# LiWentomng/BoxInstSeg

Measured on AMD Instinct MI355X. Metric: pairwise+projection loss fwd+bwd images/sec @2x800x1024x32inst, higher is better.
Workload: dtype f32; 1 GPU; BoxInst R-50 FPN loss path, 2x800x1024 synthetic batch, 32 instances, 1xMI355X per rank (BASELINE configs[1]); instances=32, launch=eager, input_sets=8, parallelism=replicas x1 (no exchange step inside the path)

## Files before the change

### boxinstseg_amd/csrc/fused_eval.hip

```cpp
#include "loss_common.hpp"
#include "dynamic_head_device.hpp"
#include <algorithm>
#include <atomic>
#include <cstdlib>
#include <cstring>
#include <cmath>
#include <ctime>

namespace bxi {

constexpr int kWaves = 4;
constexpr int kSRows = 8;
constexpr int kSBlk = kWaves * kSRows;
constexpr int kChunkC = 256;
constexpr int kMaxDilFused = 4;
#ifndef BXI_SPIN_LIMIT
#define BXI_SPIN_LIMIT 4000000
#endif
constexpr int kSpinLimit = BXI_SPIN_LIMIT;
constexpr unsigned kFlagSingle = BXI_EVAL_SINGLE_LAUNCH, kFlagTwo = BXI_EVAL_TWO_LAUNCHES, kFlagRows8 = BXI_EVAL_TILE_ROWS_8, kFlagRows4 = BXI_EVAL_TILE_ROWS_4,
                   kFlagShared = BXI_EVAL_SHARED_DEVICE, kFlagTargetsReady = BXI_EVAL_TARGETS_READY, kFlagGiveUp = BXI_EVAL_WAITS_GIVE_UP;
constexpr int kBoxCap = 1024;
constexpr int kBoxSplit = 8;
constexpr int kNtStreamFromMB = 20;
constexpr int kLongFrom = 96;
constexpr unsigned int kMaxTag = 0x0fffffffu;
constexpr int kAcc2Split = 8, kAcc2Stride = 16;
constexpr int kAcc1Words = 64;
constexpr int kMaxInst = 65536;
constexpr int kOneOcc = 4;
constexpr int kLongOcc = 3;
constexpr int kPrepOcc = 5;
#ifdef BXI_WAITLOG
static __device__ unsigned int g_waitlog[16];
#define BXI_WL(site, spins) do { if ((spins) > 1000 && (threadIdx.x & 63) == 0) atomicMax(&g_waitlog[site], (unsigned int)(spins)); } while (0)
#else
#define BXI_WL(site, spins) do {} while (0)
#endif
constexpr unsigned kFaultCounts = 1u, kFaultFinisher = 2u;
constexpr unsigned long long kCountFault = 1ull << 39, kSumwFault = 1ull << 62, kDiceFault = 1ull << 33;

#ifdef BXI_TRACE
#ifdef BXI_TRACE_LIGHT
#define BXI_TW(kid, idx, ph)                                                                                  \
    do {                                                                                                      \
        if (((ph) == 0 || (ph) == 7 || (kid) >= 2) && (threadIdx.x & 63) == 0 && g_trace && (idx) >= 0 && (idx) < ::bxi::kTraceBlocks) \
            g_trace[((size_t)(kid) * ::bxi::kTraceBlocks + (idx)) * ::bxi::kTracePhases + (ph)] = wall_clock64(); \
    } while (0)
#else
#define BXI_TW(kid, idx, ph)                                                                                  \
    do {                                                                                                      \
        if ((threadIdx.x & 63) == 0 && g_trace && (idx) >= 0 && (idx) < ::bxi::kTraceBlocks)                  \
            g_trace[((size_t)(kid) * ::bxi::kTraceBlocks + (idx)) * ::bxi::kTracePhases + (ph)] = wall_clock64(); \
    } while (0)
#endif
#else
#define BXI_TW(kid, idx, ph) do {} while (0)
#endif

constexpr int kSleepTab = 16, kSleepPred = 16, kSleepWords = 8, kSleepSumw = 8, kSleepLead = 4, kSleepFin = 2;

#define BXI_RLX __ATOMIC_RELAXED
#define BXI_AGENT __HIP_MEMORY_SCOPE_AGENT

__device__ __forceinline__ void add_f32(float* p, float v) {
    (void)__builtin_amdgcn_global_atomic_fadd_f32((__attribute__((address_space(1))) float*)p, v);
}

typedef unsigned int u4v __attribute__((ext_vector_type(4)));
__device__ __forceinline__ u4v load16_past(const void* p) {
    u4v v;
    asm volatile("global_load_dwordx4 %0, %1, off sc1\n\ts_waitcnt vmcnt(0)" : "=&v"(v) : "v"(p) : "memory");
    return v;
}
__device__ __forceinline__ void load16_past_x4(const void* p0, const void* p1, const void* p2, const void* p3, u4v& a, u4v& b, u4v& c, u4v& d) {
    asm volatile("global_load_dwordx4 %0, %4, off sc1\n\tglobal_load_dwordx4 %1, %5, off sc1\n\tglobal_load_dwordx4 %2, %6, off sc1\n\t"
                 "global_load_dwordx4 %3, %7, off sc1\n\ts_waitcnt vmcnt(0)"
                 : "=&v"(a), "=&v"(b), "=&v"(c), "=&v"(d) : "v"(p0), "v"(p1), "v"(p2), "v"(p3) : "memory");
}
__device__ __forceinline__ void load8_past_x2(const void* p0, const void* p1, unsigned long long& a, unsigned long long& b) {
    asm volatile("global_load_dwordx2 %0, %2, off sc1\n\tglobal_load_dwordx2 %1, %3, off sc1\n\ts_waitcnt vmcnt(0)" : "=&v"(a), "=&v"(b) : "v"(p0), "v"(p1) : "memory");
}
__device__ __forceinline__ void load16_past_x3(const void* p0, const void* p1, const void* p2, u4v& a, u4v& b, u4v& c) {
    asm volatile("global_load_dwordx4 %0, %3, off sc1\n\tglobal_load_dwordx4 %1, %4, off sc1\n\tglobal_load_dwordx4 %2, %5, off sc1\n\ts_waitcnt vmcnt(0)"
                 : "=&v"(a), "=&v"(b), "=&v"(c) : "v"(p0), "v"(p1), "v"(p2) : "memory");
}
__device__ __forceinline__ void load16_past_x5(const void* p0, const void* p1, const void* p2, const void* p3, const void* p4, u4v& a, u4v& b, u4v& c, u4v& d,
                                               u4v& e) {
    asm volatile("global_load_dwordx4 %0, %5, off sc1\n\tglobal_load_dwordx4 %1, %6, off sc1\n\tglobal_load_dwordx4 %2, %7, off sc1\n\t"
                 "global_load_dwordx4 %3, %8, off sc1\n\tglobal_load_dwordx4 %4, %9, off sc1\n\ts_waitcnt vmcnt(0)"
                 : "=&v"(a), "=&v"(b), "=&v"(c), "=&v"(d), "=&v"(e) : "v"(p0), "v"(p1), "v"(p2), "v"(p3), "v"(p4) : "memory");
}
__device__ __forceinline__ u4v load16_past_epoch(const void* p, const unsigned int* epoch, unsigned int& ep_word) {
    u4v v;
    asm volatile("global_load_dword %1, %3, %4\n\tglobal_load_dwordx4 %0, %2, off sc1\n\ts_waitcnt vmcnt(0)"
                 : "=&v"(v), "=&v"(ep_word) : "v"(p), "v"(0), "s"(epoch) : "memory");
    return v;
}
__device__ __forceinline__ void load16_past_x5_epoch(const void* p0, const void* p1, const void* p2, const void* p3, const void* p4, const unsigned int* epoch,
                                                     u4v& a, u4v& b, u4v& c, u4v& d, u4v& e, unsigned int& ep_word) {
    asm volatile("global_load_dword %5, %11, %12\n\tglobal_load_dwordx4 %0, %6, off sc1\n\tglobal_load_dwordx4 %1, %7, off sc1\n\t"
                 "global_load_dwordx4 %2, %8, off sc1\n\tglobal_load_dwordx4 %3, %9, off sc1\n\tglobal_load_dwordx4 %4, %10, off sc1\n\t"
                 "s_waitcnt vmcnt(0)"
                 : "=&v"(a), "=&v"(b), "=&v"(c), "=&v"(d), "=&v"(e), "=&v"(ep_word)
                 : "v"(p0), "v"(p1), "v"(p2), "v"(p3), "v"(p4), "v"(0), "s"(epoch)
                 : "memory");
}
#define BXI_PW_LD(i) "global_load_dword %[v" #i "], %[o" #i "], %[b] sc1\n\t"
#define BXI_PW_OUT(i) [v##i] "=&v"(v[i])
#define BXI_PW_IN(i) [o##i] "v"(off[i])
template <int N>
__device__ __forceinline__ void load_words_past(const unsigned int* base_in, const uint32_t (&off)[N], uint32_t (&v)[N]) {
    static_assert(N >= 5 && N <= 12, "R + D of the tile kernels");
    const unsigned long long b64 = reinterpret_cast<unsigned long long>(base_in);
    const unsigned int* base = reinterpret_cast<const unsigned int*>(
        ((unsigned long long)(unsigned int)__builtin_amdgcn_readfirstlane((int)(b64 >> 32)) << 32) | (unsigned int)__builtin_amdgcn_readfirstlane((int)b64));
    if constexpr (N == 5)
        asm volatile(BXI_PW_LD(0) BXI_PW_LD(1) BXI_PW_LD(2) BXI_PW_LD(3) BXI_PW_LD(4) "s_waitcnt vmcnt(0)"
                     : BXI_PW_OUT(0), BXI_PW_OUT(1), BXI_PW_OUT(2), BXI_PW_OUT(3), BXI_PW_OUT(4)
                     : BXI_PW_IN(0), BXI_PW_IN(1), BXI_PW_IN(2), BXI_PW_IN(3), BXI_PW_IN(4), [b] "s"(base) : "memory");
    else if constexpr (N == 6)
        asm volatile(BXI_PW_LD(0) BXI_PW_LD(1) BXI_PW_LD(2) BXI_PW_LD(3) BXI_PW_LD(4) BXI_PW_LD(5) "s_waitcnt vmcnt(0)"
                     : BXI_PW_OUT(0), BXI_PW_OUT(1), BXI_PW_OUT(2), BXI_PW_OUT(3), BXI_PW_OUT(4), BXI_PW_OUT(5)
                     : BXI_PW_IN(0), BXI_PW_IN(1), BXI_PW_IN(2), BXI_PW_IN(3), BXI_PW_IN(4), BXI_PW_IN(5), [b] "s"(base) : "memory");
    else if constexpr (N == 7)
        asm volatile(BXI_PW_LD(0) BXI_PW_LD(1) BXI_PW_LD(2) BXI_PW_LD(3) BXI_PW_LD(4) BXI_PW_LD(5) BXI_PW_LD(6) "s_waitcnt vmcnt(0)"
                     : BXI_PW_OUT(0), BXI_PW_OUT(1), BXI_PW_OUT(2), BXI_PW_OUT(3), BXI_PW_OUT(4), BXI_PW_OUT(5), BXI_PW_OUT(6)
                     : BXI_PW_IN(0), BXI_PW_IN(1), BXI_PW_IN(2), BXI_PW_IN(3), BXI_PW_IN(4), BXI_PW_IN(5), BXI_PW_IN(6), [b] "s"(base) : "memory");
    else if constexpr (N == 8)
// ... 419 lines not shown
                int t = 0;
                t += (yin && x0 + 0 < iw) ? denorm_u8(v[ch].x, s, m) : 0;
                t += (yin && x0 + 1 < iw) ? denorm_u8(v[ch].y, s, m) : 0;
                t += (yin && x0 + 2 < iw) ? denorm_u8(v[ch].z, s, m) : 0;
                t += (yin && x0 + 3 < iw) ? denorm_u8(v[ch].w, s, m) : 0;
                sum[ch] = t;
            }
        }
#pragma unroll
        for (int ch = 0; ch < 3; ++ch) part[(wv * 3 + ch) * 64 + lane] = sum[ch];
        BXI_TW(0, tix, 1);
        lds_barrier();
        BXI_TW(0, tix, 2);
        if (wv < 3) {
            int px[3];
#pragma unroll
            for (int ch = 0; ch < 3; ++ch)
                px[ch] = (part[(0 * 3 + ch) * 64 + lane] + part[(1 * 3 + ch) * 64 + lane] + part[(2 * 3 + ch) * 64 + lane] +
                          part[(3 * 3 + ch) * 64 + lane]) >> 4;
            fch[wv * 64 + lane] = lab_f(lut, wv, px[0], px[1], px[2]);
        }
        BXI_TW(0, tix, 3);
        lds_barrier();
        BXI_TW(0, tix, 4);
        if (wv == 3 && act) {
            const double f0 = fch[lane], f1 = fch[64 + lane], f2 = fch[128 + lane];
            store4_through(reinterpret_cast<float*>(ws.lab4 + ((int64_t)b * h + r) * w + c), (float)__dadd_rn(__dmul_rn(116.0, f1), -16.0),
                           (float)__dmul_rn(500.0, __dadd_rn(f0, -f1)), (float)__dmul_rn(200.0, __dadd_rn(f1, -f2)), __uint_as_float(ws.ep));
        }
#pragma unroll
        for (int ch = 0; ch < 3; ++ch) v[ch] = nx[ch];
    }
}


template <int C, bool REL>
__global__ __launch_bounds__(256, 7) void head_prep_kernel(PoolArgs pa, int n_pool, int n_items, InstArgs a, int dil, int R, Ws ws_in, LossState st,
                                                            float* __restrict__ g_logits, DynArgs da, const float* __restrict__ params,
                                                            float* __restrict__ logits_out, int ready, unsigned int key) {
    extern __shared__ __attribute__((aligned(16))) unsigned char smem[];
    Ws ws = with_tag(ws_in);
    const int n_tab = ((a.N + 64) / 64 + kWaves - 1) / kWaves;
    const int blk = (int)blockIdx.x;
    const int tix = blk * kWaves + (int)(threadIdx.x >> 6);
    (void)tix;
    if (blk < n_tab) {
        const int k = blk * kWaves + (int)(threadIdx.x >> 6);
        if (64 * k <= a.N) table_wave(a, pa.meta, dil, R, ws, st, k, true, ready, key);
    } else if (blk < n_tab + n_pool) {
        double* lut = reinterpret_cast<double*>(smem);
        double* fch = lut + 256;
        int* part = reinterpret_cast<int*>(fch + 3 * 64);
        pool_block(pa, ws, blk - n_tab, n_pool, n_items, lut, part, fch, tix);
    } else {
        const int tiles_x = (da.W + kYC - 1) / kYC, tiles_y = (da.H + kHeadR - 1) / kHeadR;
        int t = blk - n_tab - n_pool;
        const int tx = t % tiles_x; t /= tiles_x;
        const int ty = t % tiles_y;
        const int n = t / tiles_y;
        unsigned long long* ckeys = reinterpret_cast<unsigned long long*>(smem);
        float* otile = reinterpret_cast<float*>(ckeys + 4 * 64);
        float* ytile = otile + 2 * kHeadR * 64;
        const DynEpi ep = {ws.colpart, ws.rowkey, g_logits, ws.n_cb, ws.n_rp, 0};
        dyn_tile_forward<C, REL, 2, true, kHeadR, kYC>(da, params, logits_out, n, ty, tx, ytile, otile, ckeys, ep);
    }
}

__global__ __launch_bounds__(256) void pack_lab4_kernel(const float* __restrict__ lab, float4* __restrict__ lab4, const unsigned int* __restrict__ epoch, int B,
                                                         int64_t P) {
    const unsigned int ep = next_tag(*epoch);
    for (int64_t i = (int64_t)blockIdx.x * 256 + threadIdx.x; i < (int64_t)B * P; i += (int64_t)gridDim.x * 256) {
        const int64_t b = i / P, p = i - b * P;
        const float* src = lab + b * 3 * P + p;
        lab4[i] = make_float4(src[0], src[P], src[2 * P], __uint_as_float(ep));
    }
}

template <int D, int R> struct TG { static constexpr int RD = R + 2 * D, TW = 64 - 2 * D; };

enum { kTilesPair = 0, kTilesOne = 1, kTilesOneReady = 2 };
constexpr bool kAheadOne = true, kAheadOneReady = false, kAheadTwo = false;
constexpr bool pair_ahead(int D, int R, int kern) {
    return R == 4 && D == 2 && (kern == kTilesOne ? kAheadOne : kern == kTilesOneReady ? kAheadOneReady : kAheadTwo);
}
constexpr int kParkBytes = 8192;
constexpr size_t tile_wave_lds(int D, int R, int kern) {
    return pair_ahead(D, R, kern) && (size_t)kParkBytes > sizeof(float) * (R + 1) * 64 ? (size_t)kParkBytes : sizeof(float) * (R + 1) * 64;
}

struct Tile {
    int r0, r1, c0, c1;
    int img, n, tile_r0, tile_c0;
    int vrow, vcol;
    int hc1;
};

__device__ __forceinline__ uint32_t row_bits(int lo, int hi, int base, int n) {
    const int a = max(lo - base, 0), b = min(hi - base, n);
    if (b <= a) return 0u;
    return ((1u << b) - 1u) & ~((1u << a) - 1u);
}

__device__ __forceinline__ uint32_t spread4(uint32_t x4) { return (x4 * 0x00204081u) & 0x01010101u; }
typedef unsigned short us2v __attribute__((ext_vector_type(2)));
__device__ __forceinline__ uint32_t pk_mul_u16(uint32_t a, uint32_t b) { return __builtin_bit_cast(uint32_t, (us2v)(__builtin_bit_cast(us2v, a) * __builtin_bit_cast(us2v, b))); }
__device__ __forceinline__ uint32_t pk_mad_u16(uint32_t a, uint32_t b, uint32_t c) {
    return __builtin_bit_cast(uint32_t, (us2v)(__builtin_bit_cast(us2v, a) * __builtin_bit_cast(us2v, b) + __builtin_bit_cast(us2v, c)));
}

template <int D>
__device__ __forceinline__ float lane_plus(float v) {
    int x = __float_as_int(v);
#pragma unroll
    for (int s = 0; s < D; ++s) x = __builtin_amdgcn_mov_dpp(x, 0x134 , 0xf, 0xf, false);
    return __int_as_float(x);
}
template <int D>
__device__ __forceinline__ float lane_minus(float v) {
    int x = __float_as_int(v);
#pragma unroll
    for (int s = 0; s < D; ++s) x = __builtin_amdgcn_mov_dpp(x, 0x13C , 0xf, 0xf, false);
    return __int_as_float(x);
}

template <int D, int R, bool ONE>
__device__ __forceinline__ void slow_tile(const float* __restrict__ Lg, const float4* __restrict__ lab4, const Tile& t, float n2max, int zero_bit,
                                          int h, int w, int lane, float* gout ) {
    const int c = t.tile_c0 - D + lane;
    const bool col_owned = lane >= D && lane < 64 - D && c < t.hc1;
    float num = 0.f;
    const float4* L0p = lab4 + (int64_t)t.img * h * w;
#pragma unroll 1
    for (int j = 0; j < R; ++j) {
        const int r = t.tile_r0 + j;
        float gacc = 0.f;
        if (col_owned && r < h) {
            const bool in_p = r >= t.r0 && r < t.r1 && c >= t.c0 && c < t.c1;
            const bool val_p = r < t.vrow && c < t.vcol;
            const int64_t pi = (int64_t)r * w + c;
            const float4 lp = ONE ? f4_of(load16_past(L0p + pi)) : L0p[pi];
            const float xa = Lg[pi];
            const float ax = logsig(xa), bx = logsig(-xa);
#pragma unroll 1
            for (int k = 0; k < 8; ++k) {
                const int kk = k < 4 ? k : k + 1;
                const int r2 = r + (kk / 3 - 1) * D, c2 = c + (kk % 3 - 1) * D;
                const bool inq = r2 >= 0 && r2 < h && c2 >= 0 && c2 < w;
                uint32_t pn = 0u;
                int64_t qi = 0;
                if (inq) {
                    qi = (int64_t)r2 * w + c2;
                    const float4 lq = ONE ? f4_of(load16_past(L0p + qi)) : L0p[qi];
                    pn = n2_of(lp.x, lp.y, lp.z, lq.x, lq.y, lq.z) <= n2max ? 1u : 0u;
                }
                const bool val_q = inq && r2 < t.vrow && c2 < t.vcol;
                const bool in_q = inq && r2 >= t.r0 && r2 < t.r1 && c2 >= t.c0 && c2 < t.c1;
                const uint32_t wp = in_p ? (val_q ? pn : (uint32_t)zero_bit) : 0u;
                const uint32_t wq = in_q ? (val_p ? pn : (uint32_t)zero_bit) : 0u;
                if (inq && (wp + wq)) {
                    const float xb = Lg[qi];
                    const float ay = logsig(xb), by = logsig(-xb);
                    const float e1 = ax + ay, e0 = bx + by;
                    const float nl2 = logsig(fabsf(e1 - e0)) - fmaxf(e1, e0);
                    num += (float)wp * nl2;
                    gacc += (float)(wp + wq) * (-(expf(ay) - expf(by)) * expf(ax + bx + nl2));
                }
// ... 191 lines not shown
__device__ __forceinline__ void math_tile(const InstArgs& a, const Ws& ws, const Tile& t, float upw_warm, float n2max, int zero_bit, int n_items,
                                          int spin_limit, float& scale, bool& have_scale, float* __restrict__ g_logits, float* gbuf ,
                                          int tix, long long& fx_sum, bool& bad_out, bool arrive, const LossState& st, float* __restrict__ losses) {
    constexpr int RD = TG<D, R>::RD;
    const int lane = threadIdx.x & 63;
    const int h = a.h, w = a.w, n = t.n;
    const int64_t P = (int64_t)h * w;
    const float* Lg = a.logits + (int64_t)n * P;
    const int c = t.tile_c0 - D + lane;
    const bool col_owned = g_logits && lane >= D && lane < 64 - D && c < t.hc1;
    float x[RD];
    load_plane<D, R>(Lg, t, h, w, lane, x);
    uint32_t pearly[R + D];
    const bool early = ws.pred_any != 0u && zero_bit == 0;
    if (early) {
        const unsigned int* pp = ws.pred + (int64_t)t.img * h * w;
        const uint32_t cc = (uint32_t)min(max(c, 0), w - 1);
#pragma unroll
        for (int i = 0; i < R + D; ++i) pearly[i] = __hip_atomic_load(pp + (uint32_t)min(max(t.tile_r0 - D + i, 0), h - 1) * (uint32_t)w + cc, BXI_RLX, BXI_AGENT);
    }
    float g[R];
    float num = 0.f;
#pragma unroll
    for (int j = 0; j < R; ++j) g[j] = 0.f;
    constexpr bool PK = D % 2 == 0 && RD % 2 == 0;
    typedef float v2 __attribute__((ext_vector_type(2)));
    float pa_[PK ? 1 : RD], pb_[PK ? 1 : RD], pt_[PK ? 1 : RD], pu_[PK ? 1 : RD], aR[PK ? 1 : RD], bR[PK ? 1 : RD], tR[PK ? 1 : RD], uR[PK ? 1 : RD];
    v2 pa2[PK ? RD / 2 : 1], pb2[PK ? RD / 2 : 1], pt2[PK ? RD / 2 : 1], pu2[PK ? RD / 2 : 1], aR2[PK ? RD / 2 : 1], bR2[PK ? RD / 2 : 1],
        tR2[PK ? RD / 2 : 1], uR2[PK ? RD / 2 : 1];
    bool sat = false;
    if constexpr (PK) {
#pragma unroll
        for (int k = 0; k < RD / 2; ++k) {
            sat |= !(fabsf(x[2 * k]) <= 34.f) || !(fabsf(x[2 * k + 1]) <= 34.f);
            const float2 s0 = sig_pair(x[2 * k]), s1 = sig_pair(x[2 * k + 1]);
            pa2[k] = v2{s0.x, s1.x}; pb2[k] = v2{s0.y, s1.y};
            aR2[k] = v2{lane_plus<D>(s0.x), lane_plus<D>(s1.x)}; bR2[k] = v2{lane_plus<D>(s0.y), lane_plus<D>(s1.y)};
            pt2[k] = pa2[k] - pb2[k]; pu2[k] = pa2[k] * pb2[k]; tR2[k] = aR2[k] - bR2[k]; uR2[k] = aR2[k] * bR2[k];
        }
    } else {
#pragma unroll
    for (int j = 0; j < RD; ++j) {
        sat |= !(fabsf(x[j]) <= 34.f);
        const float2 s = sig_pair(x[j]); pa_[j] = s.x; pb_[j] = s.y; pt_[j] = s.x - s.y; pu_[j] = s.x * s.y;
        aR[j] = lane_plus<D>(pa_[j]); bR[j] = lane_plus<D>(pb_[j]); tR[j] = aR[j] - bR[j]; uR[j] = aR[j] * bR[j];
    }
    }
    const bool slow = zero_bit != 0 || __any(sat);
    constexpr bool AHEAD = pair_ahead(D, R, KERN);
    static_assert(!AHEAD || (PK && D == 2), "the packed loop only; slot numbering below: direction 0 is skipped in the first step only");
    constexpr int NSLOT = AHEAD ? 4 * ((R + D) / 2) - 1 : 0;
    constexpr int NPARK = kParkBytes / (64 * 16), NLDS = AHEAD ? (NSLOT < NPARK ? NSLOT : NPARK) : 0;
    constexpr int NREG = AHEAD ? NSLOT - NLDS : 0;
    typedef float v4 __attribute__((ext_vector_type(4)));
    v2 klg2[NREG ? NREG : 1], krc2[NREG ? NREG : 1];
    if constexpr (AHEAD) {
        if (!slow) {
            if constexpr (PK) {
                v4* park = reinterpret_cast<v4*>(gbuf) + lane;
#define BXI_AHEAD2(ip, ka, kb, qa, qb, dir)                                                                         \
                {                                                                                                   \
                    const int s = 4 * (ip) + (dir) - 1;                                                             \
                    const v2 S = pa2[ka] * qa[kb] + pb2[ka] * qb[kb];                                               \
                    const v2 lg = {__builtin_amdgcn_logf(S.x), __builtin_amdgcn_logf(S.y)};                         \
                    const v2 rc = {__builtin_amdgcn_rcpf(S.x), __builtin_amdgcn_rcpf(S.y)};                         \
                    if (s < NLDS) park[s * 64] = v4{lg.x, lg.y, rc.x, rc.y};                                        \
                    else { klg2[s < NLDS ? 0 : s - NLDS] = lg; krc2[s < NLDS ? 0 : s - NLDS] = rc; }                \
                }
#pragma unroll
                for (int ip = 0; ip < (R + D) / 2; ++ip) {
                    const int jp = ip + D / 2;
                    if (2 * ip >= D) BXI_AHEAD2(ip, ip, ip, aR2, bR2, 0)
                    BXI_AHEAD2(ip, jp, ip, aR2, bR2, 1)
                    BXI_AHEAD2(ip, ip, jp, pa2, pb2, 2)
                    BXI_AHEAD2(ip, ip, jp, aR2, bR2, 3)
                }
#undef BXI_AHEAD2
#pragma unroll
                for (int k = 0; k < NREG; ++k) asm volatile("" : "+v"(klg2[k]), "+v"(krc2[k]));
            }
            asm volatile("" ::: "memory");
        }
    }
    bool bad = false;
    const int band0 = t.tile_r0 / kSBlk, band1 = (min(t.tile_r0 + R, h) - 1) / kSBlk;
    const bool look_early = !slow && (!have_scale || (ONE && g_logits));
    unsigned long long sw_early = 0ull;
    unsigned int f0e = 0u, f1e = 0u;
    BXI_TW(1, tix, 2);
    if (!slow) {
        uint32_t pbyte[R + D];
        if (early) {
            bool all = true;
#pragma unroll
            for (int i = 0; i < R + D; ++i) { pbyte[i] = pearly[i]; all = all && (pbyte[i] >> 4) == 0u; }
            bad |= !__all(all);
        } else bad |= !pred_words<D, R, (!ONE || R == 8)>(ws, t, h, w, c, spin_limit, pbyte);
        float gq[PK ? 1 : RD], gR[PK ? 1 : RD];
        v2 gq2[PK ? RD / 2 : 1], gR2[PK ? RD / 2 : 1];
        if constexpr (PK) {
#pragma unroll
            for (int k = 0; k < RD / 2; ++k) { gq2[k] = v2{0.f, 0.f}; gR2[k] = v2{0.f, 0.f}; }
        } else {
#pragma unroll
            for (int j = 0; j < RD; ++j) { gq[j] = 0.f; gR[j] = 0.f; }
        }
        constexpr int NQ = (R + D + 3) / 4;
        uint32_t cw[4][NQ], dw[4][NQ];
        {
            uint32_t spb[4][NQ];
#pragma unroll
            for (int q4 = 0; q4 < NQ; ++q4) {
                uint32_t W = 0u;
#pragma unroll
                for (int k = 0; k < 4; ++k)
                    if (4 * q4 + k < R + D) W |= (pbyte[4 * q4 + k] & 15u) << (8 * k);
#pragma unroll
                for (int d = 0; d < 4; ++d) spb[d][q4] = (W >> d) & 0x01010101u;
            }
            const int base = t.tile_r0 - D;
            const uint32_t rows_box = row_bits(t.r0, t.r1, base, RD), rows_val = row_bits(0, min(h, t.vrow), base, RD);
            const uint32_t rows_own = row_bits(t.tile_r0, min(t.tile_r0 + R, h), base, RD);
            const uint32_t X1 = rows_box & rows_val, X2 = (rows_box >> D) & rows_val, X3 = rows_box & (rows_val >> D);
            const uint32_t X1O = X1 & rows_own, X2OD = X2 & (rows_own >> D), X3O = X3 & rows_own;
            const int cl = t.tile_c0 - D + lane, cr = cl + D, cv = min(w, t.vcol);
            const bool inR = lane + D < 64;
            const uint32_t fa = cl >= t.c0 && cl < t.c1, fv = cl >= 0 && cl < cv, fo = lane >= D && lane < 64 - D && cl < t.hc1;
            const uint32_t faR = inR && cr >= t.c0 && cr < t.c1, fvR = inR && cr >= 0 && cr < cv, foR = inR && lane < 64 - 2 * D && cr < t.hc1;
            const uint32_t p1 = fa & fvR, q1 = faR & fv, s1 = fa & fv;
            const uint32_t kp = p1 * 0x10001u, kq = q1 * 0x10001u, ks = s1 * 0x10001u, kpq = kp + kq;
            const uint32_t kpo = (p1 & fo) * 0x10001u, kqo = (q1 & foR) * 0x10001u, kso = (s1 & fo) * 0x10001u, kpqo = kpo + kqo;
#pragma unroll
            for (int q4 = 0; q4 < NQ; ++q4) {
                const uint32_t b1 = spread4((X1 >> (4 * q4)) & 15u), b2 = spread4((X2 >> (4 * q4)) & 15u), b3 = spread4((X3 >> (4 * q4)) & 15u);
                const uint32_t b1o = spread4((X1O >> (4 * q4)) & 15u), b2o = spread4((X2OD >> (4 * q4)) & 15u), b3o = spread4((X3O >> (4 * q4)) & 15u);
                cw[0][q4] = pk_mul_u16(spb[0][q4] & b1, kpq);
                cw[1][q4] = pk_mad_u16(spb[1][q4] & b2, kp, pk_mul_u16(spb[1][q4] & b3, kq));
                cw[2][q4] = pk_mul_u16((spb[2][q4] & b3) + (spb[2][q4] & b2), ks);
                cw[3][q4] = pk_mad_u16(spb[3][q4] & b3, kp, pk_mul_u16(spb[3][q4] & b2, kq));
                dw[0][q4] = pk_mul_u16(spb[0][q4] & b1o, kpqo);
                dw[1][q4] = pk_mad_u16(spb[1][q4] & b2o, kpo, pk_mul_u16(spb[1][q4] & b3o, kqo));
                dw[2][q4] = pk_mul_u16((spb[2][q4] & b3o) + (spb[2][q4] & b2o), kso);
                dw[3][q4] = pk_mad_u16(spb[3][q4] & b3o, kpo, pk_mul_u16(spb[3][q4] & b2o, kqo));
            }
        }
        BXI_TW(1, tix, 3);
        if (look_early) {
            if (!have_scale) sw_early = __hip_atomic_load(ws.sumw, BXI_RLX, BXI_AGENT);
            if (ONE && g_logits) {
                f0e = __hip_atomic_load(&ws.bandflag[(int64_t)n * ws.n_cb + band0], BXI_RLX, BXI_AGENT);
                f1e = __hip_atomic_load(&ws.bandflag[(int64_t)n * ws.n_cb + band1], BXI_RLX, BXI_AGENT);
            }
        }
        const v4* park2 = reinterpret_cast<const v4*>(gbuf) + lane;
        (void)park2;
#define BXI_PAIR(i, ra, rb, qa, qb, qt, qu, dir, GA, GB)                                                            \
        {                                                                                                           \
            const float gw = (float)((cw[dir][(i) >> 2] >> (8 * ((i) & 3))) & 255u);                                \
            const float nw = (float)((dw[dir][(i) >> 2] >> (8 * ((i) & 3))) & 255u);                                \
            const float S = pa_[ra] * qa[rb] + pb_[ra] * qb[rb];                                \
            num -= nw * __builtin_amdgcn_logf(S);                                            \
            const float mm = gw * __builtin_amdgcn_rcpf(S);                                                         \
            GA -= mm * qt[rb] * pu_[ra];                                                                            \
            GB -= mm * pt_[ra] * qu[rb];                                                                            \
        }
        if constexpr (PK) {
            v2 num2 = {0.f, 0.f};
#define BXI_PAIR2(ip, ka, kb, qa, qb, qt, qu, dir, GA, GB)                                                          \
            {                                                                                                       \
                const uint32_t cwd = cw[dir][(2 * (ip)) >> 2] >> (8 * ((2 * (ip)) & 3));                              \
                const uint32_t dwd = dw[dir][(2 * (ip)) >> 2] >> (8 * ((2 * (ip)) & 3));                              \
                const v2 gw = {(float)(cwd & 255u), (float)((cwd >> 8) & 255u)};                                      \
                const v2 nw = {(float)(dwd & 255u), (float)((dwd >> 8) & 255u)};                                      \
                v2 lg, rc;                                                                                            \
                if constexpr (AHEAD) {                                                \
                    const int s = 4 * (ip) + (dir) - 1;                                                               \
                    if (s < NLDS) { const v4 pk = park2[s * 64]; lg = v2{pk.x, pk.y}; rc = v2{pk.z, pk.w}; }          \
                    else { lg = klg2[s < NLDS ? 0 : s - NLDS]; rc = krc2[s < NLDS ? 0 : s - NLDS]; }                  \
                } else {                                                                                              \
                    const v2 S = pa2[ka] * qa[kb] + pb2[ka] * qb[kb];                                                 \
                    lg = v2{__builtin_amdgcn_logf(S.x), __builtin_amdgcn_logf(S.y)};                                  \
                    rc = v2{__builtin_amdgcn_rcpf(S.x), __builtin_amdgcn_rcpf(S.y)};                                  \
                }                                                                                                     \
                num2 -= nw * lg;                                                                                      \
                const v2 mm = gw * rc;                                                                                \
                GA -= mm * qt[kb] * pu2[ka];                                                                          \
                GB -= mm * pt2[ka] * qu[kb];                                                                          \
            }
#pragma unroll
            for (int ip = 0; ip < (R + D) / 2; ++ip) {
                const int jp = ip + D / 2;
                if (2 * ip >= D) BXI_PAIR2(ip, ip, ip, aR2, bR2, tR2, uR2, 0, gq2[ip], gR2[ip])
                BXI_PAIR2(ip, jp, ip, aR2, bR2, tR2, uR2, 1, gq2[jp], gR2[ip])
                BXI_PAIR2(ip, ip, jp, pa2, pb2, pt2, pu2, 2, gq2[ip], gq2[jp])
                BXI_PAIR2(ip, ip, jp, aR2, bR2, tR2, uR2, 3, gq2[ip], gR2[jp])
                if (2 * ip >= D) {
                    const float fromL0 = lane_minus<D>(gR2[ip].x), fromL1 = lane_minus<D>(gR2[ip].y);
                    g[2 * ip - D] = gq2[ip].x + (lane >= D ? fromL0 : 0.f);
                    g[2 * ip + 1 - D] = gq2[ip].y + (lane >= D ? fromL1 : 0.f);
                }
            }
#undef BXI_PAIR2
            num = num2.x + num2.y;
        } else {
#pragma unroll
        for (int i = 0; i < R + D; ++i) {
            const int j = i + D;
            if (i >= D) BXI_PAIR(i, i, i, aR, bR, tR, uR, 0, gq[i], gR[i])
            BXI_PAIR(i, j, i, aR, bR, tR, uR, 1, gq[j], gR[i])
            BXI_PAIR(i, i, j, pa_, pb_, pt_, pu_, 2, gq[i], gq[j])
            BXI_PAIR(i, i, j, aR, bR, tR, uR, 3, gq[i], gR[j])
            if (i >= D) {
                const float fromL = lane_minus<D>(gR[i]);
                g[i - D] = gq[i] + (lane >= D ? fromL : 0.f);
            }
        }
        }
        num *= 0.69314718055994531f;
#undef BXI_PAIR
    } else {
        if (ONE) {
            uint32_t pbyte[R + D];
            bad |= !pred_words<D, R, (!ONE || R == 8)>(ws, t, h, w, c, spin_limit, pbyte);
        }
        slow_tile<D, R, ONE>(Lg, ws.lab4, t, n2max, zero_bit, h, w, lane, gbuf);
        num = gbuf[R * 64 + lane];
#pragma unroll
        for (int j = 0; j < R; ++j) g[j] = gbuf[j * 64 + lane];
    }
    BXI_TW(1, tix, 5);
    num = wave_total_f32(num);
    fx_sum += (long long)(num * kNumScale);
    if (arrive) tile_wave_arrives(ws, a.N, tix, fx_sum, bad);
    bool bands_ok = !ONE || !g_logits;
    if (look_early) {
        if (!have_scale && (sw_early >> 63) != 0ull) {
            if (sw_early & kSumwFault) bad = true;
            have_scale = true;
            scale = upw_warm / fmaxf((float)(double)(sw_early & (kSumwFault - 1ull)), 1.f);
        }
        if (ONE && g_logits) bands_ok = f0e == ws.ep && f1e == ws.ep;
    }
    if (!have_scale || !bands_ok) {
        double total_w = 0.0;
        bool ok = false;
        for (int spins = 0; spins <= spin_limit; ++spins) {
            unsigned int f0 = ws.ep, f1 = ws.ep;
            if (!bands_ok) {
                f0 = __hip_atomic_load(&ws.bandflag[(int64_t)n * ws.n_cb + band0], BXI_RLX, BXI_AGENT);
                f1 = __hip_atomic_load(&ws.bandflag[(int64_t)n * ws.n_cb + band1], BXI_RLX, BXI_AGENT);
            }
            if (!have_scale) {
                if (zero_bit) { total_w = total_weight_all_pairs(a, ws); have_scale = true; }
                else have_scale = counts_complete(ws, n_items, &total_w, &bad);
                if (have_scale) scale = upw_warm / fmaxf((float)total_w, 1.f);
            }
            bands_ok = f0 == ws.ep && f1 == ws.ep;
            if (have_scale && bands_ok) { ok = true; BXI_WL(5, spins); break; }
            __builtin_amdgcn_s_sleep(kSleepSumw);
        }
        bad |= !ok;
        have_scale = true;
    }
    BXI_TW(1, tix, 4);
    if (arrive && bad) {
        if (g_logits) {
            float* G = g_logits + (int64_t)n * P;
#pragma unroll
            for (int j = 0; j < R; ++j) {
                const int r = t.tile_r0 + j;
                if (col_owned && r < h) G[(int64_t)r * w + c] = __int_as_float(0x7fc00000);
            }
        }
        if (lane == 0) {
            atomicOr(ws.fault, kFaultCounts);
            if (st.status) atomicOr(st.status, (int)kFaultCounts);
            losses[0] = __int_as_float(0x7fc00000); losses[1] = losses[0];
        }
    } else if (g_logits) {
        char* G = reinterpret_cast<char*>(g_logits + (int64_t)n * P);
#pragma unroll
        for (int j = 0; j < R; ++j) {
            const int r = t.tile_r0 + j;
            if (col_owned && r < h) add_f32(reinterpret_cast<float*>(G + (uint32_t)(r * w + c) * 4u), g[j] * scale);
        }
    }
    BXI_TW(1, tix, 6);
    bad_out |= bad;
}

__device__ __forceinline__ void block_sum4(float (&v)[4], float* red ) {
#pragma unroll
    for (int k = 0; k < 4; ++k) v[k] = wave_total_f32(v[k]);
    __syncthreads();
    if ((threadIdx.x & 63) == 0)
#pragma unroll
        for (int k = 0; k < 4; ++k) red[(threadIdx.x >> 6) * 4 + k] = v[k];
    __syncthreads();
#pragma unroll
    for (int k = 0; k < 4; ++k) v[k] = (red[k] + red[4 + k]) + (red[8 + k] + red[12 + k]);
}
__device__ __forceinline__ float sigmoid_acc(float x) { return 1.f / (1.f + expf(-x)); }

template <bool ONE>
__device__ __forceinline__ void leader_block(const InstArgs& a, int dil, Ws ws , const LossState& st, int n, float upp,
                                             float* __restrict__ g_logits, unsigned char* smem, float* red, int spin_limit) {
    const int h = a.h, w = a.w, tid = threadIdx.x;
    float* xs = reinterpret_cast<float*>(smem);
    float* ys = xs + w;
    int* carg = reinterpret_cast<int*>(ys + h);
    int* rarg = carg + w;
    int4 e;
    bool waited;
    if (ONE) {
        const int lane = tid & 63;
        waited = false;
// ... 178 lines not shown
                                   (unsigned long long)(unsigned int)((pred_cnt[0] + pred_cnt[1]) + (pred_cnt[2] + pred_cnt[3])),
                               BXI_RLX, BXI_AGENT);
    }
    BXI_TW(2, pid, 1);
}

template <bool ONE>
__device__ __forceinline__ void reducer_role(const Ws& ws, int zero_bit, int n_items, int spin_limit) {
    if (threadIdx.x >= 64 || zero_bit || n_items <= 0) return;
    if (!(table_complete<ONE>(ws, 0, spin_limit) && reduce_counts(ws, n_items, spin_limit)) && threadIdx.x == 0) atomicOr(ws.fault, kFaultCounts);
}

template <bool ONE>
__device__ __forceinline__ void finisher_role(const InstArgs& a, const Ws& ws, const LossState& st, float upp, float upw, float warmup, int zero_bit, int n_items,
                                              int spin_limit, int R, int n_tile_waves, float* __restrict__ losses) {
    const int lane = (int)(threadIdx.x & 63), wave = (int)(threadIdx.x >> 6);
    const int N = a.N;
    __builtin_amdgcn_s_setprio(3);
    BXI_TW(3, 0, 0);
    __shared__ double fin_d[kWaves];
    __shared__ int fin_i[kWaves];
    __shared__ float fin_f;
    __shared__ int fin_ok, fin_flt, fin_b[kWaves];
    bool ok = true, flt0 = false;
    double total_w = 0.0;
    float dsum = 0.f;
    int spins = 0;
    if (spin_limit < 0) ok = false;
    if (wave == 0) {
        if (!table_complete<ONE>(ws, N, spin_limit)) ok = false;
        for (int b0 = 0; b0 < N && ok; b0 += 64) {
            while (!dice_round(ws, N, b0, &dsum, &flt0)) {
                if (++spins > spin_limit) { ok = false; break; }
                __builtin_amdgcn_s_sleep(kSleepFin);
            }
        }
        if (zero_bit) total_w = total_weight_all_pairs(a, ws);
        else
            while (ok && !counts_complete(ws, n_items, &total_w, &flt0)) {
                if (++spins > spin_limit) ok = false;
                __builtin_amdgcn_s_sleep(kSleepFin);
            }
        BXI_WL(8, spins);
        if (lane == 0) { fin_f = dsum; fin_d[0] = total_w; fin_ok = ok ? 1 : 0; fin_flt = flt0 ? 1 : 0; }
    }
    __syncthreads();
    ok = fin_ok != 0; dsum = fin_f; total_w = fin_d[0];
    __syncthreads();
    long long mine = 0;
    unsigned int fault_seen = (ok ? 0u : kFaultFinisher) | (fin_flt ? kFaultCounts : 0u);
    spins = 0;
    for (; ok;) {
        mine = 0;
        int arrived = 0;
        bool flt = false;
        {
            const int n_words = (N < 64 ? N : 64) * kAcc2Split;
            const int i0 = threadIdx.x, i1 = threadIdx.x + 256;
            unsigned long long x0 = 0ull, x1 = 0ull;
            if (n_words > 256) load8_past_x2(ws.acc2 + (size_t)(i0 < n_words ? i0 : 0) * kAcc2Stride, ws.acc2 + (size_t)(i1 < n_words ? i1 : 0) * kAcc2Stride, x0, x1);
            else x0 = __hip_atomic_load(ws.acc2 + (size_t)(i0 < n_words ? i0 : 0) * kAcc2Stride, BXI_RLX, BXI_AGENT);
            if (i0 >= n_words) x0 = 0ull;
            if (i1 >= n_words) x1 = 0ull;
#pragma unroll
            for (int k = 0; k < 2; ++k) {
                const unsigned long long x = k ? x1 : x0;
                arrived += (int)(x >> 52);
                mine += (long long)(x & ((1ull << 52) - 1ull)) - ((long long)(x >> 52) << 24);
                flt |= (x & (3ull << 50)) != 0ull;
            }
        }
        if (threadIdx.x == 0) fault_seen |= __hip_atomic_load(ws.fault, BXI_RLX, BXI_AGENT);
        arrived = wave_total_i32(arrived);
        const bool anyflt = __any(flt);
        if (lane == 0) { fin_i[wave] = arrived; fin_b[wave] = anyflt ? 1 : 0; }
        __syncthreads();
        const bool all = (fin_i[0] + fin_i[1]) + (fin_i[2] + fin_i[3]) == n_tile_waves;
        if ((fin_b[0] | fin_b[1]) | (fin_b[2] | fin_b[3])) fault_seen |= kFaultCounts;
        __syncthreads();
        if (all) break;
        if (++spins > spin_limit) { ok = false; break; }
    }
    BXI_WL(10, spins);
    if (threadIdx.x == 0) fault_seen |= __hip_atomic_load(ws.fault, BXI_RLX, BXI_AGENT);
    const double wsum = wave_total_f64((double)mine);
    if (lane == 0) fin_d[wave] = wsum;
    __syncthreads();
    if (threadIdx.x >= 64) return;
    const double num = (fin_d[0] + fin_d[1]) + (fin_d[2] + fin_d[3]);
    const unsigned int status = (unsigned int)__builtin_amdgcn_readfirstlane((int)(fault_seen | (ok ? 0u : kFaultFinisher)));
    if (lane == 0) {
        const float denom = fmaxf((float)total_w, 1.f);
        float l0 = dsum / (float)N;
        float l1 = (float)((num / (double)kNumScale) / (double)denom) * warmup;
        if (status) { l0 = __int_as_float(0x7fc00000); l1 = l0; }
        losses[0] = l0; losses[1] = l1;
        if (st.scale) { st.scale[0] = warmup / denom; st.scale[1] = warmup; st.applied[0] = upp; st.applied[1] = upw; }
        if (st.status) { st.status[0] = (int)status; if (ONE) st.status[1] = R; }
        if (st.iter) atomicAdd(st.iter, 1.0f);
        if (ws.ep != kMaxTag) *ws.epoch = ws.ep;
    }
    if (ws.ep == kMaxTag) {
        uint4* z = reinterpret_cast<uint4*>(ws.epoch);
        const size_t n16 = ws.ws_n16;
        for (size_t i = lane; i < n16; i += 64) z[i] = make_uint4(0u, 0u, 0u, 0u);
    }
    BXI_TW(3, 0, 1);
}

template <int D, int R, bool ONE, int KERN>
__device__ __forceinline__ void tile_role(const InstArgs& a, const ValidCells& vc, const Ws& ws, float upw_warm, float n2max, int zero_bit, int n_items, int spin_limit,
                                          float* __restrict__ g_logits, unsigned char* smem, int tblk, int n_tb, const LossState& st, float* __restrict__ losses) {
    const int lane = (int)(threadIdx.x & 63), wave = (int)(threadIdx.x >> 6);
    const int N = a.N;
    const int wid = tblk * kWaves + wave, nwaves = n_tb * kWaves;
    BXI_TW(1, wid, 0);
    int4 e0, e1 = make_int4(0, 0, 0, 0), eN = make_int4(0, 0, 0, 0);
    bool ok;
    if (ONE && R == 8 && N >= 64) {
        ok = false;
        const bool want1 = 64 + lane < N;
        for (int spins = 0; spins <= spin_limit; ++spins) {
            u4v v0, vN, v1;
            load16_past_x3(ws.tab + lane, ws.tab + N, ws.tab + (want1 ? 64 + lane : N), v0, vN, v1);
            if (__all(v0.w == ws.ep && vN.w == ws.ep && v1.w == ws.ep)) {
                e0 = make_int4((int)v0.x, (int)v0.y, (int)v0.z, (int)v0.w); eN = make_int4((int)vN.x, (int)vN.y, (int)vN.z, (int)vN.w);
                if (want1) e1 = make_int4((int)v1.x, (int)v1.y, (int)v1.z, (int)v1.w);
                ok = true;
                BXI_WL(1, spins);
                break;
            }
            __builtin_amdgcn_s_sleep(kSleepTab);
        }
    } else {
        ok = tab_entry<ONE>(ws, lane, lane <= N, spin_limit, e0);
        if (N >= 64) ok = ok && tab_entry<ONE>(ws, N, true, spin_limit, eN);
        if (N > 64) ok = ok && tab_entry<ONE>(ws, 64 + lane, 64 + lane < N, spin_limit, e1);
    }
    if (!ok) { tile_wave_arrives(ws, N, wid, 0, true); return; }
    const int total = N < 64 ? __builtin_amdgcn_readlane(e0.x, N < 64 ? N : 0) : __builtin_amdgcn_readfirstlane(eN.x);
    float* gbuf = reinterpret_cast<float*>(smem + wave * tile_wave_lds(D, R, KERN));
    float scale = 0.f;
    bool have_scale = false, bad = false;
    long long fx_sum = 0;
    const bool may_arrive_early = ONE && ws.ep != kMaxTag;
    bool arrived = false;
    for (int ti = wid; ti < total && !bad; ti += nwaves) {
        Tile t;
        if (!locate_tile<D, R, ONE>(ws, vc, N, e0, e1, ti, a.h, a.w, spin_limit, t)) { bad = true; break; }
        BXI_TW(1, wid, 1);
        const bool last = may_arrive_early && ti + nwaves >= total;
        math_tile<D, R, ONE, KERN>(a, ws, t, upw_warm, n2max, zero_bit, n_items, spin_limit, scale, have_scale, g_logits, gbuf, wid, fx_sum, bad, last, st, losses);
        arrived = last;
    }
    if (!arrived) tile_wave_arrives(ws, N, wid, fx_sum, bad);
    BXI_TW(1, wid, 7);
}

struct PrepTail {
    int ready;
    unsigned int key;
};

__global__ __launch_bounds__(256, kPrepOcc) void prep_kernel(PoolArgs pa, int n_pool, int n_items, InstArgs a, int dil, int R, Ws ws_in, LossState st,
                                                       float* __restrict__ g_logits, int vec, int pool_first, PrepTail tl) {
    extern __shared__ __attribute__((aligned(16))) unsigned char smem[];
// ... 573 lines not shown
```

Before: 120,100 images/s.

## Compute loss before arrival and defer gradient pass; precompute row/col masks early

In the single-kernel R=4,D=2 tile path, the pairwise loss numerator is now computed in a first pass so the wave can publish its arrival to the finisher sooner. The gradient accumulation runs in a second pass after the arrival. The box/validity/ownership masks are built before waiting on the prediction words, so less work remains after the wait. In exchange, the parked logits/coefficients are read twice and more registers stay live across the arrival. Trace macros are extended for tile phases.

```diff
diff --git a/boxinstseg_amd/csrc/fused_eval.hip b/boxinstseg_amd/csrc/fused_eval.hip
--- a/boxinstseg_amd/csrc/fused_eval.hip
+++ b/boxinstseg_amd/csrc/fused_eval.hip
@@ -42,9 +42,14 @@
 
 #ifdef BXI_TRACE
 #ifdef BXI_TRACE_LIGHT
+#ifdef BXI_TRACE_TILES
+#define BXI_TW_TILES(kid, ph) ((kid) == 1 && ((ph) == 2 || (ph) == 3 || (ph) == 5 || (ph) == 6))
+#else
+#define BXI_TW_TILES(kid, ph) false
+#endif
 #define BXI_TW(kid, idx, ph)                                                                                  \
     do {                                                                                                      \
-        if (((ph) == 0 || (ph) == 7 || (kid) >= 2) && (threadIdx.x & 63) == 0 && g_trace && (idx) >= 0 && (idx) < ::bxi::kTraceBlocks) \
+        if (((ph) == 0 || (ph) == 7 || (kid) >= 2 || BXI_TW_TILES(kid, ph)) && (threadIdx.x & 63) == 0 && g_trace && (idx) >= 0 && (idx) < ::bxi::kTraceBlocks) \
             g_trace[((size_t)(kid) * ::bxi::kTraceBlocks + (idx)) * ::bxi::kTracePhases + (ph)] = wall_clock64(); \
     } while (0)
 #else
@@ -630,6 +635,14 @@
 constexpr bool kAheadOne = true, kAheadOneReady = false, kAheadTwo = false;
 constexpr bool pair_ahead(int D, int R, int kern) {
     return R == 4 && D == 2 && (kern == kTilesOne ? kAheadOne : kern == kTilesOneReady ? kAheadOneReady : kAheadTwo);
+}
+constexpr bool kLossFirstOne = true, kLossFirstOneReady = false;
+constexpr bool kMasksAheadOne = true, kMasksAheadOneReady = false, kMasksAheadTwo = false;
+constexpr bool loss_first(int D, int R, int kern) {
+    return pair_ahead(D, R, kern) && (kern == kTilesOne ? kLossFirstOne : kern == kTilesOneReady ? kLossFirstOneReady : false);
+}
+constexpr bool masks_ahead(int D, int R, int kern) {
+    return R == 4 && D == 2 && (kern == kTilesOne ? kMasksAheadOne : kern == kTilesOneReady ? kMasksAheadOneReady : kMasksAheadTwo);
 }
 constexpr int kParkBytes = 8192;
 constexpr size_t tile_wave_lds(int D, int R, int kern) {
@@ -987,11 +1000,46 @@
             asm volatile("" ::: "memory");
         }
     }
+    constexpr bool MASKS = masks_ahead(D, R, KERN);
+    constexpr int NQ = (R + D + 3) / 4;
+    uint32_t Mp[2][MASKS ? NQ : 1];
+    if constexpr (MASKS) {
+        if (!slow) {
+            const int base = t.tile_r0 - D;
+            const uint32_t rows_box = row_bits(t.r0, t.r1, base, RD), rows_val = row_bits(0, min(h, t.vrow), base, RD);
+            const uint32_t rows_own = row_bits(t.tile_r0, min(t.tile_r0 + R, h), base, RD);
+            const uint32_t X1 = rows_box & rows_val, X2 = (rows_box >> D) & rows_val, X3 = rows_box & (rows_val >> D);
+            const uint32_t X1O = X1 & rows_own, X2OD = X2 & (rows_own >> D), X3O = X3 & rows_own;
+            const int cl = t.tile_c0 - D + lane, cr = cl + D, cv = min(w, t.vcol);
+            const bool inR = lane + D < 64;
+            const uint32_t fa = cl >= t.c0 && cl < t.c1, fv = cl >= 0 && cl < cv, fo = lane >= D && lane < 64 - D && cl < t.hc1;
+            const uint32_t faR = inR && cr >= t.c0 && cr < t.c1, fvR = inR && cr >= 0 && cr < cv, foR = inR && lane < 64 - 2 * D && cr < t.hc1;
+            const uint32_t p1 = fa & fvR, q1 = faR & fv, s1 = fa & fv;
+            const uint32_t kp = p1 * 0x10001u, kq = q1 * 0x10001u, ks = s1 * 0x10001u, kpq = kp + kq;
+            const uint32_t kpo = (p1 & fo) * 0x10001u, kqo = (q1 & foR) * 0x10001u, kso = (s1 & fo) * 0x10001u, kpqo = kpo + kqo;
+#pragma unroll
+            for (int q4 = 0; q4 < NQ; ++q4) {
+                const uint32_t b1 = spread4((X1 >> (4 * q4)) & 15u), b2 = spread4((X2 >> (4 * q4)) & 15u), b3 = spread4((X3 >> (4 * q4)) & 15u);
+                const uint32_t b1o = spread4((X1O >> (4 * q4)) & 15u), b2o = spread4((X2OD >> (4 * q4)) & 15u), b3o = spread4((X3O >> (4 * q4)) & 15u);
+                const uint32_t c0 = pk_mul_u16(b1, kpq), c1 = pk_mad_u16(b2, kp, pk_mul_u16(b3, kq));
+                const uint32_t c2 = pk_mul_u16(b3 + b2, ks), c3 = pk_mad_u16(b3, kp, pk_mul_u16(b2, kq));
+                const uint32_t d0 = pk_mul_u16(b1o, kpqo), d1 = pk_mad_u16(b2o, kpo, pk_mul_u16(b3o, kqo));
+                const uint32_t d2 = pk_mul_u16(b3o + b2o, kso), d3 = pk_mad_u16(b3o, kpo, pk_mul_u16(b2o, kqo));
+                Mp[0][q4] = c0 | (d0 << 2) | (c1 << 4) | (d1 << 6);
+                Mp[1][q4] = c2 | (d2 << 2) | (c3 << 4) | (d3 << 6);
+                asm volatile("" : "+v"(Mp[0][q4]), "+v"(Mp[1][q4]));
+            }
+        }
+    }
     bool bad = false;
     const int band0 = t.tile_r0 / kSBlk, band1 = (min(t.tile_r0 + R, h) - 1) / kSBlk;
     const bool look_early = !slow && (!have_scale || (ONE && g_logits));
     unsigned long long sw_early = 0ull;
     unsigned int f0e = 0u, f1e = 0u;
+    constexpr bool LOSS_FIRST = loss_first(D, R, KERN);
+    const bool two_pass = LOSS_FIRST && !slow && arrive;
+    v2 gq2[PK ? RD / 2 : 1], gR2[PK ? RD / 2 : 1];
+    uint32_t cw[4][NQ], dw[4][NQ];
     BXI_TW(1, tix, 2);
     if (!slow) {
         uint32_t pbyte[R + D];
@@ -1002,7 +1050,6 @@
             bad |= !__all(all);
         } else bad |= !pred_words<D, R, (!ONE || R == 8)>(ws, t, h, w, c, spin_limit, pbyte);
         float gq[PK ? 1 : RD], gR[PK ? 1 : RD];
-        v2 gq2[PK ? RD / 2 : 1], gR2[PK ? RD / 2 : 1];
         if constexpr (PK) {
 #pragma unroll
             for (int k = 0; k < RD / 2; ++k) { gq2[k] = v2{0.f, 0.f}; gR2[k] = v2{0.f, 0.f}; }
@@ -1010,9 +1057,21 @@
 #pragma unroll
             for (int j = 0; j < RD; ++j) { gq[j] = 0.f; gR[j] = 0.f; }
         }
-        constexpr int NQ = (R + D + 3) / 4;
-        uint32_t cw[4][NQ], dw[4][NQ];
-        {
+        if constexpr (MASKS) {
+#pragma unroll
+            for (int q4 = 0; q4 < NQ; ++q4) {
+                uint32_t W = 0u;
+#pragma unroll
+                for (int k = 0; k < 4; ++k)
+                    if (4 * q4 + k < R + D) W |= (pbyte[4 * q4 + k] & 15u) << (8 * k);
+#pragma unroll
+                for (int d = 0; d < 4; ++d) {
+                    const uint32_t sel = pk_mul_u16((W >> d) & 0x01010101u, 0x00030003u);
+                    cw[d][q4] = (Mp[d >> 1][q4] >> (4 * (d & 1))) & sel;
+                    dw[d][q4] = (Mp[d >> 1][q4] >> (4 * (d & 1) + 2)) & sel;
+                }
+            }
+        } else {
             uint32_t spb[4][NQ];
 #pragma unroll
             for (int q4 = 0; q4 < NQ; ++q4) {
@@ -1092,6 +1151,31 @@
                 GA -= mm * qt[kb] * pu2[ka];                                                                          \
                 GB -= mm * pt2[ka] * qu[kb];                                                                          \
             }
+#define BXI_LOSS2(ip, dir)                                                                                          \
+            {                                                                                                       \
+                const uint32_t dwd = dw[dir][(2 * (ip)) >> 2] >> (8 * ((2 * (ip)) & 3));                              \
+                const v2 nw = {(float)(dwd & 255u), (float)((dwd >> 8) & 255u)};                                      \
+                const int s = 4 * (ip) + (dir) - 1;                                                                   \
+                const v2 lg = s < NLDS ? parkh[(s < NLDS ? s : 0) * 128] : klg2[s < NLDS ? 0 : s - NLDS];             \
+                num2 -= nw * lg;                                                                                      \
+            }
+            if (two_pass) {
+                if constexpr (LOSS_FIRST) {
+                    const v2* parkh = reinterpret_cast<const v2*>(gbuf) + 2 * lane;
+#pragma unroll
+                    for (int q4 = 0; q4 < NQ; ++q4)
+#pragma unroll
+                        for (int d = 0; d < 4; ++d) asm volatile("" : "+v"(dw[d][q4]));
+#pragma unroll
+                    for (int ip = 0; ip < (R + D) / 2; ++ip) {
+                        if (2 * ip >= D) BXI_LOSS2(ip, 0)
+                        BXI_LOSS2(ip, 1)
+                        BXI_LOSS2(ip, 2)
+                        BXI_LOSS2(ip, 3)
+                    }
+                    num = num2.x + num2.y;
+                }
+            } else {
 #pragma unroll
             for (int ip = 0; ip < (R + D) / 2; ++ip) {
                 const int jp = ip + D / 2;
@@ -1105,8 +1189,10 @@
                     g[2 * ip + 1 - D] = gq2[ip].y + (lane >= D ? fromL1 : 0.f);
                 }
             }
+            num = num2.x + num2.y;
+            }
 #undef BXI_PAIR2
-            num = num2.x + num2.y;
+#undef BXI_LOSS2
         } else {
 #pragma unroll
         for (int i = 0; i < R + D; ++i) {
@@ -1137,6 +1223,40 @@
     num = wave_total_f32(num);
     fx_sum += (long long)(num * kNumScale);
     if (arrive) tile_wave_arrives(ws, a.N, tix, fx_sum, bad);
+    if constexpr (LOSS_FIRST && PK) {
+        if (two_pass) {
+            const v2* parkh = reinterpret_cast<const v2*>(gbuf) + 2 * lane;
+            asm volatile("" ::: "memory");
+#pragma unroll
+            for (int q4 = 0; q4 < NQ; ++q4)
+#pragma unroll
+                for (int d = 0; d < 4; ++d) asm volatile("" : "+v"(cw[d][q4]));
+#define BXI_GRAD2(ip, ka, kb, qt, qu, dir, GA, GB)                                                                  \
+            {                                                                                                       \
+                const uint32_t cwd = cw[dir][(2 * (ip)) >> 2] >> (8 * ((2 * (ip)) & 3));                              \
+                const v2 gw = {(float)(cwd & 255u), (float)((cwd >> 8) & 255u)};                                      \
+                const int s = 4 * (ip) + (dir) - 1;                                                                   \
+                const v2 rc = s < NLDS ? parkh[(s < NLDS ? s : 0) * 128 + 1] : krc2[s < NLDS ? 0 : s - NLDS];         \
+                const v2 mm = gw * rc;                                                                                \
+                GA -= mm * qt[kb] * pu2[ka];                                                                          \
+                GB -= mm * pt2[ka] * qu[kb];                                                                          \
+            }
+#pragma unroll
+            for (int ip = 0; ip < (R + D) / 2; ++ip) {
+                const int jp = ip + D / 2;
+                if (2 * ip >= D) BXI_GRAD2(ip, ip, ip, tR2, uR2, 0, gq2[ip], gR2[ip])
+                BXI_GRAD2(ip, jp, ip, tR2, uR2, 1, gq2[jp], gR2[ip])
+                BXI_GRAD2(ip, ip, jp, pt2, pu2, 2, gq2[ip], gq2[jp])
+                BXI_GRAD2(ip, ip, jp, tR2, uR2, 3, gq2[ip], gR2[jp])
+                if (2 * ip >= D) {
+                    const float fromL0 = lane_minus<D>(gR2[ip].x), fromL1 = lane_minus<D>(gR2[ip].y);
+                    g[2 * ip - D] = gq2[ip].x + (lane >= D ? fromL0 : 0.f);
+                    g[2 * ip + 1 - D] = gq2[ip].y + (lane >= D ? fromL1 : 0.f);
+                }
+            }
+#undef BXI_GRAD2
+        }
+    }
     bool bands_ok = !ONE || !g_logits;
     if (look_early) {
         if (!have_scale && (sw_early >> 63) != 0ull) {
@@ -1481,6 +1601,7 @@
         if (++spins > spin_limit) { ok = false; break; }
     }
     BXI_WL(10, spins);
+    BXI_TW(3, 0, 2);
     if (threadIdx.x == 0) fault_seen |= __hip_atomic_load(ws.fault, BXI_RLX, BXI_AGENT);
     const double wsum = wave_total_f64((double)mine);
     if (lane == 0) fin_d[wave] = wsum;
```

Result: no change. 120,100 images/s (median of 4 runs) (+0.0%).
